# spcl/EBCC

Measured on AMD Instinct MI355X. Metric: fp32 GB/s encode+decode, 721x1440 ERA5 frames MAX_ERROR=0.5, higher is better.
Workload: dtype f32; 1 GPU; 256-frame batch 721x1440 fp32 per GPU, base_cr=30 MAX_ERROR=0.5 (BASELINE configs[1]); frames_per_gpu=256, parallelism=frames sharded over 1 GPU(s), no collective, hw_queues=4, encode_slices=3

## Files before the change

### ebcc_amd/csrc/j2k.hip

```cpp
#include <algorithm>
#include <cstring>
#include <vector>

#include "../../include/ebcc_hip.h"
#include "engine.hpp"
#include "j2k.hpp"
#include "search.hpp"

namespace ebcc {

bool j2k_create(ebcc_hip_ctx *ctx)
{
    J2kBuffers *jb = new J2kBuffers();
    ctx->j2k = jb;
    const int period = ctx->tile_period;
    std::vector<std::vector<J2kBlock>> tile_blocks((size_t) period);
    int stride = 0;
    for (int k = 0; k < period; k++) {
        jb->geoms.push_back(make_j2k_geom(ctx->height, ctx->width, tile_blocks[(size_t) k], k * ctx->height));
        stride = std::max(stride, jb->geoms.back().nblocks);
    }
    for (J2kGeom &t : jb->geoms) { t.period = period; t.stride = stride; }
    jb->geom = jb->geoms[0];
    const J2kGeom &g = jb->geom;
// ... 39 lines not shown
    ok &= (jb->cand_npass = (int *) ctx_alloc<int32_t>(ctx, 2 * F * (size_t) stride)) != nullptr;
    ok &= (jb->cand_sel = (int *) ctx_alloc<int32_t>(ctx, F)) != nullptr;
    ok &= (jb->have_rate = (int *) ctx_alloc<int32_t>(ctx, F)) != nullptr;
    ok &= (jb->rate_path = (int *) ctx_alloc<int32_t>(ctx, F * 1536 * 3)) != nullptr;
    ok &= (jb->rate_path_n = (int *) ctx_alloc<int32_t>(ctx, 2 * F)) != nullptr;
    {
        int nodes = 0;
        for (const J2kGeom &t : jb->geoms) nodes = std::max(nodes, t.tree_nodes);
        J2kBuffers::RateCache &rc = jb->rate_cache;
        rc.nodes_cap = (nodes + 3) & ~3;
        rc.cap = stride * kJ2kMaxPasses;
        rc.ok = jb->rate_path_n ? jb->rate_path_n + F : nullptr;
        ok &= (rc.mnmx = ctx_alloc<double>(ctx, F * 2)) != nullptr;
        ok &= (rc.mval = (short *) ctx_alloc<uint16_t>(ctx, F * (size_t) rc.nodes_cap)) != nullptr;
        ok &= (rc.off = (int *) ctx_alloc<int32_t>(ctx, F * (size_t) (stride + 1))) != nullptr;
        ok &= (rc.crate = ctx_alloc<uint16_t>(ctx, F * (size_t) rc.cap)) != nullptr;
        ok &= (rc.cdisto = ctx_alloc<double>(ctx, F * (size_t) rc.cap)) != nullptr;
    }
    ok &= (jb->rates = (int *) ctx_alloc<int32_t>(ctx, groups * 64 * kJ2kMaxPasses)) != nullptr;
    ok &= (jb->disto = ctx_alloc<double>(ctx, groups * 64 * kJ2kMaxPasses)) != nullptr;
    ok &= (jb->cblk_bytes = ctx_alloc<uint8_t>(ctx, groups * 64 * kJ2kCblkBytes)) != nullptr;
    ok &= (jb->stream = ctx_alloc<uint8_t>(ctx, F * jb->stream_cap)) != nullptr;
    ok &= (jb->dec_table = (int *) ctx_alloc<int32_t>(ctx, groups * 64 * 4)) != nullptr;
    ok &= (jb->dec_order = (int *) ctx_alloc<int32_t>(ctx, groups * 64 + 128)) != nullptr;
    ok &= (jb->mq_order = (int *) ctx_alloc<int32_t>(ctx, groups * 64 + 256)) != nullptr;
    ok &= (jb->jf = (J2kFrame *) ctx_alloc<uint8_t>(ctx, sizeof(J2kFrame) * F)) != nullptr;
    ok &= (jb->partial = ctx_alloc<double>(ctx, F * kPartials)) != nullptr;
    ok &= (jb->partial_u = ctx_alloc<unsigned long long>(ctx, F * kPartials)) != nullptr;
    if (!ok) return false;
    poison_alloc(jb->cblk_bytes, groups * 64 * kJ2kCblkBytes);
    poison_alloc(jb->stream, F * jb->stream_cap);
    if (stride >= 65535) { set_error("too many code-blocks"); return false; }
// ... 643 lines not shown
```

### ebcc_amd/csrc/j2k.hpp

```cpp
#pragma once

#include <vector>

#include "../../include/ebcc_hip.h"
#include "common.hpp"
#include "residual.hpp"

namespace ebcc {

constexpr int kJ2kRes = 6;
constexpr int kJ2kBands = 3 * kJ2kRes - 2;
constexpr int kJ2kMaxPlanes = 26;
constexpr int kJ2kMaxPasses = 3 * kJ2kMaxPlanes;
constexpr int kJ2kCblkBytes = 16 * 1024;
constexpr int kT1StateWords = 66 + 4 * 64;

struct J2kBand {
    int res, orient, level;
    int x0, y0, x1, y1;
    int offx, offy;
    int ncw, nch;
    int first_block;
    int expn, mant, numbps;
    float step_enc, step_dec;
// ... 95 lines not shown
    int *npass;
    float *cand_cr;
    int *cand_out;
    int *cand_npass;
    int *cand_sel;
    int *have_rate;
    int *rate_path;
    int *rate_path_n;
    struct RateCache {
        int *ok;
        double *mnmx;
        short *mval;
        int *off;
        unsigned short *crate;
        double *cdisto;
        int nodes_cap, cap;
    } rate_cache;
    uint8_t *cblk_bytes;
    uint8_t *stream;
    size_t stream_cap;
    int32_t *V;
    int *dec_table;
    int *dec_order;
    int *mq_order;
    J2kFrame *jf;
    FrameState *fs;
    double *partial;
    unsigned long long *partial_u;
};

enum T1Kernel { T1_ENCODE = 0, T1_MQ = 1, T1_RESUME = 2, T1_DECODE = 3 };
int t1_lanes_per_wave(int kernel, int total_blocks = 0);
// ... 37 lines not shown
    J2kBoxList list{};
    float *out = nullptr;
};
bool j2k_list_check(const char *who, const J2kGeom &g, size_t n_frames, const ebcc_hip_placed_box *boxes, size_t n_boxes, size_t out_floats,
                    uint8_t *keep = nullptr, J2kBoxEntry *table = nullptr, J2kPlacement *place = nullptr, int first_fused = kJ2kRes,
                    int *max_rows = nullptr, int *max_cols = nullptr);
bool j2k_boxes_as_placed(const char *who, const ebcc_hip_box *boxes, size_t n_boxes, size_t rows, size_t cols,
                         std::vector<ebcc_hip_placed_box> &placed, size_t *out_floats);
int j2k_selfcheck_div65535();

void launch_input_stats(const float *data, int n_frames, size_t n_pix, FrameState *fs, hipStream_t s);
void launch_j2k_analysis(const float *data, const J2kBuffers &jb, int n_frames, hipStream_t s);
void launch_j2k_tier1(const J2kBuffers &jb, int n_frames, hipStream_t s, bool single_kernel);
bool j2k_tier1_retry(const J2kBuffers &jb, int n_frames, const J2kFrame *host_jf, hipStream_t s);
void launch_j2k_rate(const J2kBuffers &jb, int n_frames, const int *d_active, hipStream_t s, const int *have_rate = nullptr);
void j2k_probe_hist_dump(const char *what);
void launch_j2k_rate_candidates(const J2kBuffers &jb, int n_frames, const int *d_active, hipStream_t s);
void launch_j2k_rate_publish(const J2kBuffers &jb, int n_frames, hipStream_t s);
void launch_j2k_write(const J2kBuffers &jb, int n_frames, const int *d_active, hipStream_t s);
void launch_j2k_probe_decode(const float *data, const J2kBuffers &jb, int n_frames, const int *d_active, hipStream_t s,
                             int keep_field = 1);
void launch_j2k_decode(const J2kBuffers &jb, int n_frames, hipStream_t s, const int *host_table = nullptr, const J2kRegion &region = J2kRegion{});
void launch_j2k_box_levels(const J2kBuffers &jb, int n_frames, const J2kBoxList &boxes, float *out, hipStream_t s);
void launch_j2k_fill_placed(const J2kBuffers &jb, const J2kBoxList &boxes, float *out, hipStream_t s);
void plan_decode_lanes(const int *host_table, int total, int out[4]);

}
```

### ebcc_amd/csrc/j2k_analysis.hip

```cpp
#include <array>
#include <mutex>
#include <cmath>
#include <cstdlib>
#include <vector>

#include "j2k.hpp"
#include "t1_core.hpp"
#include "t1_device.hpp"

namespace ebcc {

static int ceildivpow2(int a, int b) { return (int) (((long long) a + (1ll << b) - 1) >> b); }
static int floorlog2i(int a) { int l = 0; while (a > 1) { a >>= 1; l++; } return l; }

static const double kNormsReal[4][10] = {
    {1.000, 1.965, 4.177, 8.403, 16.90, 33.84, 67.69, 135.3, 270.6, 540.9},
    {2.022, 3.989, 8.355, 17.04, 34.27, 68.63, 137.3, 274.6, 549.0},
    {2.022, 3.989, 8.355, 17.04, 34.27, 68.63, 137.3, 274.6, 549.0},
    {2.080, 3.865, 8.307, 17.18, 34.71, 69.59, 139.3, 278.6, 557.2}};

int t1_lanes_per_wave(int kernel, int total_blocks)
{
    int t[4] = {64, 64, 4, 2};
    if (const char *e = getenv("EBCC_T1_LPW")) {
// ... 1551 lines not shown
            EBCC_HIP_CHECK(hipMemsetAsync(counters, 0, 2 * kMqClasses * sizeof(int), s));
            hipLaunchKernelGGL(k_mq_hist, dim3(ceil_div(total, 256)), dim3(256), 0, s, jb.lanerows, counters, total, (uint32_t) jb.sym_rows);
            hipLaunchKernelGGL(k_mq_offsets, dim3(1), dim3(kMqClasses), 0, s, counters);
            hipLaunchKernelGGL(k_mq_place, dim3(ceil_div((int) (groups * 64), 256)), dim3(256), 0, s, jb.lanerows, counters, jb.mq_order, total, (int) (groups * 64),
                               (uint32_t) jb.sym_rows);
            order = jb.mq_order;
        }
        hipLaunchKernelGGL(k_t1_mqrows, dim3((unsigned) groups), dim3(128), 0, s, jb.SYM, jb.lanerows, jb.blkmax, jb.cblk_len, jb.rates,
                           jb.cblk_bytes, jb.ckpt, jb.d_geom, jb.d_blocks, fs, jb.jf, total, (uint32_t) jb.sym_rows, order);
        timing_end("t1_mq", s);
    }
    timing_end("t1_encode", s);
    hipLaunchKernelGGL(k_distortion, dim3(g.stride, n_frames), dim3(256), 0, s, jb.Q6, jb.SPS, jb.numbps, jb.totalpasses,
                       jb.disto, nmsedec_luts(s), jb.d_geom, jb.d_blocks, fs);
    EBCC_HIP_LAUNCH_CHECK();
}

bool j2k_tier1_retry(const J2kBuffers &jb, int n_frames, const J2kFrame *host_jf, hipStream_t s)
{
    bool need = false;
    for (int f = 0; f < n_frames; f++) need |= (host_jf[f].overflow & 2) != 0;
    if (!need) return false;
    hipLaunchKernelGGL(k_jf_reset, dim3(ceil_div(n_frames, 64)), dim3(64), 0, s, jb.jf, n_frames);
    launch_j2k_tier1(jb, n_frames, s, true);
    return true;
}

constexpr int kFwdT = 64;
__global__ __launch_bounds__(kFwdT) void k_j2k_cols_fwd_top(const float *__restrict__ data, float *__restrict__ B, const J2kGeom *geom,
                                                             const FrameState *fs)
// ... 204 lines not shown
```

### ebcc_amd/csrc/j2k_rate.hip

```cpp
#include <cfloat>
#include <cmath>
#include <cstdlib>
#include <mutex>

#include "j2k.hpp"
#include "t1_core.hpp"
#include "t1_device.hpp"

namespace ebcc {

int j2k_inverse_dwt(float *B, const int32_t *V, const float *data, const J2kBuffers &jb, int n_frames, const FrameState *fs,
                    const int *active, hipStream_t s, int keep_field, const J2kWindow *win = nullptr, float *win_out = nullptr);

namespace {

constexpr int kMainHeaderBytes = 135;
constexpr int kRateTrieNodes = 1536;
#ifndef EBCC_RATE_THREADS
#define EBCC_RATE_THREADS 512
#endif
constexpr int kRateThreads = EBCC_RATE_THREADS;
constexpr int kWriteThreads = 256;

__device__ inline int floorlog2d(int a) { return a > 1 ? 31 - __clz(a) : 0; }
// ... 77 lines not shown
                int inc = floorlog2d(seglen) + 1 - (3 + floorlog2d(n));
                if (inc < 0) inc = 0;
                for (int k = 0; k < inc; k++) bio.bit(1);
                bio.bit(0);
                bio.bits((unsigned) seglen, 3 + inc + floorlog2d(n));
                bytes += seglen;
            }
    }
    bio.flush();
    *body = bytes;
    return bio.n;
}

__host__ __device__ inline size_t rate_off_bytes(int nblocks) { return ((size_t) (nblocks + 1) * 4 + 15) & ~(size_t) 15; }
__host__ __device__ inline size_t rate_path_bytes(int nblocks) { return (size_t) nblocks * 2 * 8 * 3 + (((size_t) nblocks + 7) & ~(size_t) 7); }

__host__ __device__ inline size_t rate_lds_bytes(int nblocks, int nodes)
{
    return 2 * ((((size_t) nblocks * 2 + 7) / 8) * 8) + (size_t) nodes * 16 + (size_t) nblocks * 20 + 128;
}

struct RateLds {
    short *npass;
    Trees t;
    short *mval0;
    short *prev;
    int *firstinc;
    unsigned int *raw;
    int *leafbits;
    __device__ static size_t bytes(int nblocks, int nodes)
// ... 80 lines not shown
}

struct PassTab {
    const int *rates;
    const double *disto;
    const __attribute__((address_space(3))) double *l_disto;
    const __attribute__((address_space(3))) unsigned short *l_rate;
    const __attribute__((address_space(3))) int *l_off;
    bool lds;
    template <bool LDS> __device__ int rate(int base, int p) const { if constexpr (LDS) return l_rate[base + p]; else return rates[base + p]; }
    template <bool LDS> __device__ double dist(int base, int p) const { if constexpr (LDS) return l_disto[base + p]; else return disto[base + p]; }
    template <bool LDS> __device__ int base_of(int b) const { if constexpr (LDS) return l_off[b]; else return b * kJ2kMaxPasses; }
};

template <bool LDS>
__device__ inline int walk_block(const PassTab &pt, const int *totalpasses, int gid0, int b, double thresh, unsigned long long &m0,
                                 unsigned long long &m1, int from = 0, int n_in = 0)
{
    if (from == 0) m0 = m1 = 0;
    int tp;
    if constexpr (LDS) tp = pt.l_off[b + 1] - pt.l_off[b]; else tp = totalpasses[gid0 + b];
    const int base = pt.base_of<LDS>(b);
    int n = n_in;
    if (thresh < 0) return tp;
    int rbase = 0;
    double dbase = 0;
    if (n_in > 0) { rbase = pt.rate<LDS>(base, n_in - 1); dbase = pt.dist<LDS>(base, n_in - 1); }
    for (int p = from; p < tp; p++) {
        const int rp = pt.rate<LDS>(base, p);
        const double dp = pt.dist<LDS>(base, p);
        unsigned int dr;
        double dd;
        if (n == 0) { dr = (unsigned int) rp; dd = dp; }
        else { dr = (unsigned int) (rp - rbase); dd = dp - dbase; }
        bool take;
        if (!dr) take = dd != 0;
        else {
            const double tdr = thresh * (double) dr;
            if (dd >= tdr * 1.00000000001) take = true;
            else if (thresh >= 1e-4 && dd <= tdr * 0.99999999999) take = false;
            else take = thresh - (dd / dr) < DBL_EPSILON;
        }
        if (take) {
            n = p + 1; rbase = rp; dbase = dp;
            if (p < 64) m0 |= 1ull << p; else m1 |= 1ull << (p - 64);
        }
    }
    return n;
}

__device__ inline double next_up(double x)
{
    long long u = __double_as_longlong(x);
    if (x == 0.0) return __longlong_as_double(1ll);
    u += x > 0.0 ? 1 : -1;
    return __longlong_as_double(u);
}
__device__ inline double next_down(double x) { return -next_up(-x); }
__device__ inline double take_limit(double s)
{
    double t = s + DBL_EPSILON;
    for (int k = 0; k < 8 && (t - s) < DBL_EPSILON; k++) t = next_up(t);
    for (int k = 0; k < 8; k++) { const double d = next_down(t); if ((d - s) < DBL_EPSILON) break; t = d; }
    return t;
}
template <bool LDS>
__device__ inline void walk_interval(const PassTab &pt, const int *totalpasses, int gid0, int b, unsigned long long m0, unsigned long long m1,
                                     int from, int n_in, double tlo, double thi, double &A, double &B)
{
    int tp;
    if constexpr (LDS) tp = pt.l_off[b + 1] - pt.l_off[b]; else tp = totalpasses[gid0 + b];
    const int base = pt.base_of<LDS>(b);
    int n = n_in, rbase = 0;
    double dbase = 0;
    if (n_in > 0) { rbase = pt.rate<LDS>(base, n_in - 1); dbase = pt.dist<LDS>(base, n_in - 1); }
    A = -DBL_MAX; B = DBL_MAX;
    const bool coarse = tlo >= 1e-4;
    for (int p = from; p < tp; p++) {
        const int rp = pt.rate<LDS>(base, p);
        const double dp = pt.dist<LDS>(base, p);
        const unsigned int dr = n == 0 ? (unsigned int) rp : (unsigned int) (rp - rbase);
        const double dd = n == 0 ? dp : dp - dbase;
        const bool taken = p < 64 ? (m0 >> p) & 1ull : (m1 >> (p - 64)) & 1ull;
        if (dr) {
            const double fdr = (double) dr;
            if (coarse && dd > thi * fdr * 1.000000001) {
                if (!taken) A = DBL_MAX;
            } else if (coarse && dd < tlo * fdr * 0.999999999) {
                if (taken) B = -DBL_MAX;
            } else {
                const double lim = take_limit(dd / fdr);
                if (taken) B = lim < B ? lim : B; else A = lim > A ? lim : A;
            }
        } else if (taken != (dd != 0)) { A = DBL_MAX; B = -DBL_MAX; }
        if (taken) { n = p + 1; rbase = rp; dbase = dp; }
    }
}

template <int NT, bool LDS>
__device__ void make_layer_impl(const J2kGeom &g, RateLds &L, const int *totalpasses, const PassTab &pt, int gid0, double thresh, int lane,
                                unsigned long long *path, const unsigned char *frozen)
{
    for (int b = lane; b < g.nblocks; b += NT) {
        if (frozen && frozen[b]) continue;
        unsigned long long m0, m1;
        const int n = walk_block<LDS>(pt, totalpasses, gid0, b, thresh, m0, m1);
        L.npass[b] = (short) n;
        if (path) { path[b] = m0; path[g.nblocks + b] = m1; }
    }
    __syncthreads();
}

template <int NT>
__device__ void make_layer(const J2kGeom &g, RateLds &L, const int *totalpasses, const PassTab &pt, int gid0, double thresh, int lane,
                           unsigned long long *path = nullptr, const unsigned char *frozen = nullptr)
{
    if (pt.lds) make_layer_impl<NT, true>(g, L, totalpasses, pt, gid0, thresh, lane, path, frozen);
    else make_layer_impl<NT, false>(g, L, totalpasses, pt, gid0, thresh, lane, path, frozen);
}

template <int NT>
// ... 141 lines not shown
            }
            if (found < 0) { count += (T - p + 7) >> 3; break; }
            count += found + 1 + 1;
            p += 8 * (found + 1) + 7;
            if (p >= T) break;
        }
        if (hdr_out && wl == 0) hdr_out[r] = count - count_before;
    }
    if (wl == 0) atomicAdd(s_sum, body + count);
    __syncthreads();
    const int total = *s_sum;
    __syncthreads();
    return total;
}

__global__ __launch_bounds__(kRateThreads) void k_rate(const int *__restrict__ numbps, const int *__restrict__ totalpasses,
                                                        const int *__restrict__ rates, const double *__restrict__ disto,
                                                        int *__restrict__ npass_out, const J2kGeom *geom, J2kFrame *jf,
                                                        const FrameState *fs, const int *active, int pass_capacity,
                                                        int *__restrict__ path_bytes, int *__restrict__ path_n,
                                                        const float *cand_cr, int *cand_out, size_t cand_stride, const int *have_rate,
                                                        J2kBuffers::RateCache cache)
{
    extern __shared__ unsigned char lds_raw[];
    __shared__ int s_sum, s_changed;
#ifdef EBCC_RATE_PROFILE
    const long long t_start = wall_clock64();
#endif
    __shared__ double s_min[kRateThreads / 64], s_max[kRateThreads / 64];
    __shared__ double s_td[5];
// ... 26 lines not shown
        for (int i = lane; i < g.tree_nodes; i += kRateThreads) L.mval0[i] = c_mval[i];
        __syncthreads();
    } else {
        trees_static<kRateThreads>(g, L, numbps, gid0, lane);
        if (record) for (int i = lane; i < g.tree_nodes; i += kRateThreads) c_mval[i] = L.mval0[i];
    }
#ifdef EBCC_RATE_PROFILE
    t_s[1] = wall_clock64() - t_start;
#endif
    for (int b = lane; b < g.nblocks; b += kRateThreads) L.prev[b] = -1;
    __shared__ int s_fit;
    unsigned char *extra = lds_raw + ((rate_lds_bytes(g.nblocks, g.tree_nodes) + 15) & ~(size_t) 15);
    int *l_off = (int *) extra;
    unsigned long long *p_cur = (unsigned long long *) (extra + rate_off_bytes(g.nblocks));
    unsigned long long *p_lo = p_cur + 2 * g.nblocks, *p_hi = p_lo + 2 * g.nblocks;
    unsigned char *frozen = (unsigned char *) (p_hi + 2 * g.nblocks);
    double *l_disto = (double *) (frozen + (((size_t) g.nblocks + 7) & ~(size_t) 7));
    for (int b = lane; b < g.nblocks; b += kRateThreads) frozen[b] = 0;
    if (cached) {
        for (int b = lane; b <= g.nblocks; b += kRateThreads) l_off[b] = c_off[b];
        if (lane == 0) { const int running = c_off[g.nblocks]; s_fit = running <= pass_capacity ? running : -1; }
    } else {
        __shared__ int s_scan[kRateThreads / 64];
        int running = 0;
        for (int base = 0; base < g.nblocks; base += kRateThreads) {
            const int b = base + lane;
            const int tp = b < g.nblocks ? totalpasses[gid0 + b] : 0;
            int x = tp;
            for (int d = 1; d < 64; d <<= 1) { const int y = __shfl_up(x, d); if ((lane & 63) >= d) x += y; }
            if ((lane & 63) == 63) s_scan[lane >> 6] = x;
            __syncthreads();
            int before = running, tot = 0;
            for (int w = 0; w < kRateThreads / 64; w++) { const int v = s_scan[w]; if (w < (lane >> 6)) before += v; tot += v; }
            if (b < g.nblocks) l_off[b] = before + x - tp;
            running += tot;
            __syncthreads();
        }
        if (lane == 0) { l_off[g.nblocks] = running; s_fit = running <= pass_capacity ? running : -1; }
        __syncthreads();
        if (record) for (int b = lane; b <= g.nblocks; b += kRateThreads) c_off[b] = l_off[b];
    }
    __syncthreads();
#ifdef EBCC_RATE_PROFILE
    t_s[2] = wall_clock64() - t_start;
#endif
    const int n_entries = s_fit;
    unsigned short *l_rate = (unsigned short *) (l_disto + (n_entries > 0 ? n_entries : 0));
    typedef __attribute__((address_space(3))) double lds_double;
    typedef __attribute__((address_space(3))) int lds_int;
    typedef __attribute__((address_space(3))) unsigned short lds_ushort;
    PassTab pt{rates + (size_t) gid0 * kJ2kMaxPasses, disto + (size_t) gid0 * kJ2kMaxPasses, (const lds_double *) l_disto,
               (const lds_ushort *) l_rate, (const lds_int *) l_off, n_entries >= 0};
    if (pt.lds && cached) {
// ... 6 lines not shown
            const int r_ = pt.rates[idx];
            const double d_ = pt.disto[idx];
            const int b = idx / kJ2kMaxPasses, p = idx - b * kJ2kMaxPasses;
            const int o = l_off[b];
            if (p < l_off[b + 1] - o) {
                l_rate[o + p] = (unsigned short) r_;
                l_disto[o + p] = d_;
                if (record) { c_rate[o + p] = (unsigned short) r_; c_disto[o + p] = d_; }
            }
        }
        __syncthreads();
    }
#ifdef EBCC_RATE_PROFILE
    t_s[3] = wall_clock64() - t_start;
#endif
    int prev_bytes = 0;
    auto sized = [&]() -> int {
        if (lane == 0) s_changed = 0;
        __syncthreads();
        int ch = 0;
        for (int b = lane; b < g.nblocks; b += kRateThreads) { if (L.prev[b] != L.npass[b]) ch = 1; L.prev[b] = L.npass[b]; }
        if (ch) s_changed = 1;
        __syncthreads();
        if (s_changed) {
#ifdef EBCC_RATE_CHECK
            const int ref = layer_bytes<kRateThreads>(g, L, rates, gid0, lane, &s_sum);
            prev_bytes = layer_bytes_fast<kRateThreads>(g, L, rates, gid0, lane, &s_sum);
            if (ref != prev_bytes && lane == 0) { printf("rate check: frame %d fast %d serial %d\n", frame, prev_bytes, ref); }
            prev_bytes = ref;
#else
// ... 28 lines not shown
            if (sl > mx) mx = sl;
        }
    }
    for (int d = 32; d >= 1; d >>= 1) {
        const double omn = __shfl_xor(mn, d), omx = __shfl_xor(mx, d);
        mn = omn < mn ? omn : mn; mx = omx > mx ? omx : mx;
    }
    if ((lane & 63) == 0) { s_min[lane >> 6] = mn; s_max[lane >> 6] = mx; }
    __syncthreads();
    for (int i = 0; i < kRateThreads / 64; i++) { mn = s_min[i] < mn ? s_min[i] : mn; mx = s_max[i] > mx ? s_max[i] : mx; }
    if (record) {
        __threadfence();
        __syncthreads();
        if (lane == 0) {
            cache.mnmx[2 * frame] = mn; cache.mnmx[2 * frame + 1] = mx;
            if (pt.lds) { __threadfence(); __hip_atomic_store(&cache.ok[frame], 1, __ATOMIC_RELEASE, __HIP_MEMORY_SCOPE_AGENT); }
        }
    }
    }

#ifdef EBCC_RATE_PROFILE
    long long t_setup = wall_clock64() - t_start, t_ml = 0, t_sz = 0, t_replay_end = 0, t_tail = 0, t_loop_end = 0; int n_it = 0, n_real = 0, n_replayed = 0, n_tail = 0;
#define RP_T0 const long long rp0 = wall_clock64()
#define RP_ADD(acc) acc += wall_clock64() - rp0
#else
#define RP_T0
#define RP_ADD(acc)
#endif
    double good = -1;
    bool converged = false;
    if (rate > 0.0f) {
// ... 14 lines not shown
#ifdef EBCC_RATE_PROFILE
                n_replayed++;
#endif
                const int bytes = trie[3 * cur];
                const int f = (long long) bytes <= maxlen;
                if (f) { hi = thresh; stable = thresh; bytes_hi = bytes; hi_from_rec = true; hi_seen = false; }
                else { lo = thresh; bytes_lo = bytes; lo_from_rec = true; lo_seen = false; }
                parent = cur; pdir = f;
                const int nxt = trie[3 * cur + 1 + f];
                cur = nxt > 0 ? nxt : -1;
                continue;
            }
#ifdef EBCC_RATE_PROFILE
            if (!t_replay_end) t_replay_end = wall_clock64();
#endif
            if (hi_from_rec) { make_layer<kRateThreads>(g, L, totalpasses, pt, gid0, hi, lane, p_hi); hi_seen = true; hi_from_rec = false; }
            if (lo_from_rec) { make_layer<kRateThreads>(g, L, totalpasses, pt, gid0, lo, lane, p_lo); lo_seen = true; lo_from_rec = false; }
            { RP_T0; make_layer<kRateThreads>(g, L, totalpasses, pt, gid0, thresh, lane, p_cur, frozen); RP_ADD(t_ml); }
            if (lane == 0) s_nun = 0;
            int at_lo = lo_seen, at_hi = hi_seen;
            for (int b = lane; b < g.nblocks; b += kRateThreads) {
                if (frozen[b]) continue;
                if (p_cur[b] != p_lo[b] || p_cur[g.nblocks + b] != p_lo[g.nblocks + b]) at_lo = 0;
                if (p_cur[b] != p_hi[b] || p_cur[g.nblocks + b] != p_hi[g.nblocks + b]) at_hi = 0;
            }
            at_lo = __syncthreads_and(at_lo);
            at_hi = __syncthreads_and(at_hi);
            int bytes;
            if (at_lo) bytes = bytes_lo;
            else if (at_hi) bytes = bytes_hi;
            else { RP_T0; bytes = sized(); RP_ADD(t_sz); }
#ifdef EBCC_RATE_PROFILE
            n_it++; n_real += (at_lo || at_hi) ? 0 : s_changed;
#endif
            const bool fits = (long long) bytes <= maxlen;
            if (record && n_nodes < kRateTrieNodes && (parent >= 0 || n_nodes == 0)) {
                if (lane == 0) {
                    trie[3 * n_nodes] = bytes; trie[3 * n_nodes + 1] = 0; trie[3 * n_nodes + 2] = 0;
                    if (parent >= 0) trie[3 * parent + 1 + pdir] = n_nodes;
                    path_n[frame] = n_nodes + 1;
                }
                parent = n_nodes++; pdir = fits;
            } else {
                parent = -1;
            }
            if (fits) bytes_hi = bytes; else bytes_lo = bytes;
            if (fits) { hi = thresh; stable = thresh; hi_seen = true; } else { lo = thresh; lo_seen = true; }
            unsigned long long *end = fits ? p_hi : p_lo;
            int same = lo_seen && hi_seen;
            for (int b = lane; b < g.nblocks; b += kRateThreads) {
                if (frozen[b]) continue;
                end[b] = p_cur[b]; end[g.nblocks + b] = p_cur[g.nblocks + b];
                if (lo_seen && hi_seen && p_lo[b] == p_hi[b] && p_lo[g.nblocks + b] == p_hi[g.nblocks + b]) frozen[b] = 1;
                else {
                    same = 0;
                    const int k = atomicAdd(&s_nun, 1);
                    if (k < 64) s_list[k] = b;
                }
            }
            if (__syncthreads_and(same)) { converged = true; break; }
            if (lo_seen && hi_seen && s_nun <= 64) {
                RP_T0;
                if (lane < 64) {
                    const int nb = g.nblocks, b = lane < s_nun ? s_list[lane] : -1;
                    double tlo = lo, thi = hi, tprev = prev, tstable = stable, tthresh = thresh;
                    int ti = i, tn = n_nodes, tparent = parent, tpdir = pdir, status = 0;
                    int from = 0, n_in = 0;
                    unsigned long long c0 = 0, c1 = 0;
                    if (b >= 0) {
                        const unsigned long long d0 = p_lo[b] ^ p_hi[b], d1 = p_lo[nb + b] ^ p_hi[nb + b];
                        from = d0 ? __builtin_ctzll(d0) : (d1 ? 64 + __builtin_ctzll(d1) : 0);
                        if (from > 0) {
                            c0 = from >= 64 ? p_lo[b] : p_lo[b] & ((1ull << from) - 1ull);
                            c1 = from > 64 ? p_lo[nb + b] & ((1ull << (from - 64)) - 1ull) : 0ull;
                            n_in = c1 ? 128 - __builtin_clzll(c1) : (c0 ? 64 - __builtin_clzll(c0) : 0);
                        }
                    }
                    double a_lo = -DBL_MAX, b_lo = DBL_MAX, a_hi = -DBL_MAX, b_hi = DBL_MAX;
                    if (b >= 0) {
                        if (pt.lds) {
                            walk_interval<true>(pt, totalpasses, gid0, b, p_lo[b], p_lo[nb + b], from, n_in, tlo, thi, a_lo, b_lo);
                            walk_interval<true>(pt, totalpasses, gid0, b, p_hi[b], p_hi[nb + b], from, n_in, tlo, thi, a_hi, b_hi);
                        } else {
                            walk_interval<false>(pt, totalpasses, gid0, b, p_lo[b], p_lo[nb + b], from, n_in, tlo, thi, a_lo, b_lo);
                            walk_interval<false>(pt, totalpasses, gid0, b, p_hi[b], p_hi[nb + b], from, n_in, tlo, thi, a_hi, b_hi);
                        }
                    }
                    (void) c0; (void) c1;
                    for (int j = i + 1; j < 128; j++) {
                        const double t = (tlo + thi) / 2;
                        if (t == tprev) { tthresh = t; break; }
                        const int all_lo = __all(b < 0 || (t >= a_lo && t < b_lo));
                        const int all_hi = __all(b < 0 || (t >= a_hi && t < b_hi));
                        if (!all_lo && !all_hi) { status = 1; break; }
                        tthresh = t; tprev = t; ti = j;
                        const int bytes = all_lo ? bytes_lo : bytes_hi;
                        const bool fits = (long long) bytes <= maxlen;
                        if (record && tn < kRateTrieNodes && (tparent >= 0 || tn == 0)) {
                            if (lane == 0) {
                                trie[3 * tn] = bytes; trie[3 * tn + 1] = 0; trie[3 * tn + 2] = 0;
// ... 16 lines not shown
                i = s_ti[0]; n_nodes = s_ti[1]; parent = s_ti[2]; pdir = s_ti[3];
                const int status = s_ti[4];
                __syncthreads();
                RP_ADD(t_tail);
#ifdef EBCC_RATE_PROFILE
                n_tail++;
#endif
                if (status == 0) break;
            }
        }
        good = stable == 0 ? thresh : stable;
    }
#ifdef EBCC_RATE_PROFILE
    t_loop_end = wall_clock64();
#endif
    if (!converged) make_layer<kRateThreads>(g, L, totalpasses, pt, gid0, good, lane);
    const int body = sized();
    for (int b = lane; b < g.nblocks; b += kRateThreads) npass_out[gid0 + b] = L.npass[b];
    if (lane == 0 && candidate) {
        int *o = cand_out + (size_t) (2 * frame + slot) * 3;
        o[0] = body; o[1] = kMainHeaderBytes + 12 + 2 + body + 2; o[2] = (int) (rate > 0.0f ? ceil((double) rate) : 0);
    }
    if (lane == 0 && !candidate) {
        jf[frame].body_bytes = body;
        jf[frame].stream_bytes = kMainHeaderBytes + 12 + 2 + body + 2;
        jf[frame].maxlen = (int) (rate > 0.0f ? ceil((double) rate) : 0);
#ifdef EBCC_RATE_PROFILE
        if (frame == 0) printf("k_rate frame0 setup: entry %lld, trees %lld, offsets %lld, tables %lld us\n", t_s[0] / 100, t_s[1] / 100, t_s[2] / 100, t_s[3] / 100);
        if (frame == 0) printf("k_rate frame0: setup %lld us, %d replayed steps until %lld us, make_layer %lld us, sized %lld us, computed iterations %d (real sizings %d), tail %lld us in %d visits, loop ends at %lld us, total %lld us\n",
                               t_setup / 100, n_replayed, t_replay_end ? (t_replay_end - t_start) / 100 : -1, t_ml / 100, t_sz / 100, n_it, n_real, t_tail / 100, n_tail,
                               (t_loop_end - t_start) / 100, (wall_clock64() - t_start) / 100);
// ... 534 lines not shown
    t1::decode_resume(st, DecSrc{cblk_bytes + (size_t) gid * kJ2kCblkBytes, len}, blk.w, blk.h, geom->bands[blk.band].orient, P,
                      np, r, stripe, ck, tab, ctxp);
}

size_t rate_lds(const J2kBuffers &jb)
{
    size_t n = 0;
    for (const J2kGeom &g : jb.geoms) n = std::max(n, rate_lds_bytes(g.nblocks, g.tree_nodes));
    return n;
}

}

static void rate_launch(const J2kBuffers &jb, int n_frames, const int *d_active, hipStream_t s, bool candidates, const int *have_rate)
{
    const size_t head = ((rate_lds(jb) + 15) & ~(size_t) 15) + rate_off_bytes(jb.geom.stride) + rate_path_bytes(jb.geom.stride);
    const size_t budget = 150 * 1024;
    size_t want = (size_t) jb.geom.stride * kJ2kMaxPasses;
    if (head + want * 10 + 16 > budget) want = head + 16 < budget ? (budget - head - 16) / 10 : 0;
    const size_t lds = head + want * 10 + 16;
    static std::once_flag once;
    std::call_once(once, [] {
        EBCC_HIP_CHECK(hipFuncSetAttribute((const void *) k_rate, hipFuncAttributeMaxDynamicSharedMemorySize, 150 * 1024));
    });
    hipLaunchKernelGGL(k_rate, dim3(n_frames, candidates ? 2 : 1), dim3(kRateThreads), lds, s, jb.numbps, jb.totalpasses, jb.rates,
                       jb.disto, candidates ? jb.cand_npass : jb.npass, jb.d_geom, jb.jf, jb.fs, d_active, (int) want, jb.rate_path, jb.rate_path_n,
                       candidates ? jb.cand_cr : nullptr, jb.cand_out, (size_t) jb.max_frames * (size_t) jb.geom.stride, have_rate, jb.rate_cache);
    EBCC_HIP_LAUNCH_CHECK();
}

void launch_j2k_rate(const J2kBuffers &jb, int n_frames, const int *d_active, hipStream_t s, const int *have_rate)
{
    ScopedTiming t("rate_alloc", s);
    rate_launch(jb, n_frames, d_active, s, false, have_rate);
}

void launch_j2k_rate_candidates(const J2kBuffers &jb, int n_frames, const int *d_active, hipStream_t s)
{
    rate_launch(jb, n_frames, d_active, s, true, nullptr);
}

__global__ void k_rate_publish(const int *sel, const int *cand_npass, const int *cand_out, size_t cand_stride, int *npass, J2kFrame *jf,
// ... 196 lines not shown
```

Measured before the change: 8.830 GB/s.

## Precompute per-block threshold tables for rate allocation and binary-search them

Adds a k_rate_tables kernel, launched after distortion, that walks each code-block's rate/distortion passes once. It records the threshold breakpoints at which the number of included passes changes, along with the pass count at each. The rate-allocation bisection then looks up each block's pass count by binary search in this table. This replaces re-walking every pass at every threshold iteration, and bracket indices narrow the search. The old walk path stays behind an environment variable; the cost is an extra kernel launch, extra global memory for the tables, and subtle exactness risks in the breakpoint computation.

```diff
diff --git a/ebcc_amd/csrc/j2k.hip b/ebcc_amd/csrc/j2k.hip
--- a/ebcc_amd/csrc/j2k.hip
+++ b/ebcc_amd/csrc/j2k.hip
@@ -77,8 +77,20 @@
         ok &= (rc.mnmx = ctx_alloc<double>(ctx, F * 2)) != nullptr;
         ok &= (rc.mval = (short *) ctx_alloc<uint16_t>(ctx, F * (size_t) rc.nodes_cap)) != nullptr;
         ok &= (rc.off = (int *) ctx_alloc<int32_t>(ctx, F * (size_t) (stride + 1))) != nullptr;
-        ok &= (rc.crate = ctx_alloc<uint16_t>(ctx, F * (size_t) rc.cap)) != nullptr;
-        ok &= (rc.cdisto = ctx_alloc<double>(ctx, F * (size_t) rc.cap)) != nullptr;
+        const char *e = getenv("EBCC_HIP_RATE_WALK");
+        jb->rate_walk = e && atoi(e);
+        rc.crate = nullptr; rc.cdisto = nullptr; rc.wlim = nullptr; rc.wnp = nullptr; rc.wcnt = nullptr;
+        if (jb->rate_walk) {
+            ok &= (rc.crate = ctx_alloc<uint16_t>(ctx, F * (size_t) rc.cap)) != nullptr;
+            ok &= (rc.cdisto = ctx_alloc<double>(ctx, F * (size_t) rc.cap)) != nullptr;
+        } else {
+            const size_t cnt_bytes = (F * (size_t) stride * sizeof(uint16_t) + 15) & ~(size_t) 15;
+            uint8_t *small = nullptr;
+            ok &= (rc.wlim = ctx_alloc<double>(ctx, F * (size_t) (rc.cap + stride))) != nullptr;
+            ok &= (small = ctx_alloc<uint8_t>(ctx, cnt_bytes + F * (size_t) (rc.cap + stride))) != nullptr;
+            rc.wcnt = (unsigned short *) small;
+            rc.wnp = small ? small + cnt_bytes : nullptr;
+        }
     }
     ok &= (jb->rates = (int *) ctx_alloc<int32_t>(ctx, groups * 64 * kJ2kMaxPasses)) != nullptr;
     ok &= (jb->disto = ctx_alloc<double>(ctx, groups * 64 * kJ2kMaxPasses)) != nullptr;
diff --git a/ebcc_amd/csrc/j2k.hpp b/ebcc_amd/csrc/j2k.hpp
--- a/ebcc_amd/csrc/j2k.hpp
+++ b/ebcc_amd/csrc/j2k.hpp
@@ -133,8 +133,12 @@
         int *off;
         unsigned short *crate;
         double *cdisto;
+        double *wlim;
+        unsigned char *wnp;
+        unsigned short *wcnt;
         int nodes_cap, cap;
     } rate_cache;
+    bool rate_walk;
     uint8_t *cblk_bytes;
     uint8_t *stream;
     size_t stream_cap;
@@ -202,6 +206,7 @@
 void launch_j2k_tier1(const J2kBuffers &jb, int n_frames, hipStream_t s, bool single_kernel);
 bool j2k_tier1_retry(const J2kBuffers &jb, int n_frames, const J2kFrame *host_jf, hipStream_t s);
 void launch_j2k_rate(const J2kBuffers &jb, int n_frames, const int *d_active, hipStream_t s, const int *have_rate = nullptr);
+void launch_j2k_rate_tables(const J2kBuffers &jb, int n_frames, hipStream_t s);
 void j2k_probe_hist_dump(const char *what);
 void launch_j2k_rate_candidates(const J2kBuffers &jb, int n_frames, const int *d_active, hipStream_t s);
 void launch_j2k_rate_publish(const J2kBuffers &jb, int n_frames, hipStream_t s);
diff --git a/ebcc_amd/csrc/j2k_analysis.hip b/ebcc_amd/csrc/j2k_analysis.hip
--- a/ebcc_amd/csrc/j2k_analysis.hip
+++ b/ebcc_amd/csrc/j2k_analysis.hip
@@ -1589,6 +1589,7 @@
     hipLaunchKernelGGL(k_distortion, dim3(g.stride, n_frames), dim3(256), 0, s, jb.Q6, jb.SPS, jb.numbps, jb.totalpasses,
                        jb.disto, nmsedec_luts(s), jb.d_geom, jb.d_blocks, fs);
     EBCC_HIP_LAUNCH_CHECK();
+    launch_j2k_rate_tables(jb, n_frames, s);
 }
 
 bool j2k_tier1_retry(const J2kBuffers &jb, int n_frames, const J2kFrame *host_jf, hipStream_t s)
diff --git a/ebcc_amd/csrc/j2k_rate.hip b/ebcc_amd/csrc/j2k_rate.hip
--- a/ebcc_amd/csrc/j2k_rate.hip
+++ b/ebcc_amd/csrc/j2k_rate.hip
@@ -4,6 +4,7 @@
 #include <mutex>
 
 #include "j2k.hpp"
+#include "rate_walk.hpp"
 #include "t1_core.hpp"
 #include "t1_device.hpp"
 
@@ -115,6 +116,7 @@
 
 __host__ __device__ inline size_t rate_off_bytes(int nblocks) { return ((size_t) (nblocks + 1) * 4 + 15) & ~(size_t) 15; }
 __host__ __device__ inline size_t rate_path_bytes(int nblocks) { return (size_t) nblocks * 2 * 8 * 3 + (((size_t) nblocks + 7) & ~(size_t) 7); }
+__host__ __device__ inline size_t rate_index_bytes(int nblocks) { return (((size_t) nblocks * 2 * 3 + 7) & ~(size_t) 7) + (((size_t) nblocks + 7) & ~(size_t) 7); }
 
 __host__ __device__ inline size_t rate_lds_bytes(int nblocks, int nodes)
 {
@@ -225,88 +227,15 @@
 };
 
 template <bool LDS>
-__device__ inline int walk_block(const PassTab &pt, const int *totalpasses, int gid0, int b, double thresh, unsigned long long &m0,
-                                 unsigned long long &m1, int from = 0, int n_in = 0)
-{
-    if (from == 0) m0 = m1 = 0;
-    int tp;
-    if constexpr (LDS) tp = pt.l_off[b + 1] - pt.l_off[b]; else tp = totalpasses[gid0 + b];
-    const int base = pt.base_of<LDS>(b);
-    int n = n_in;
-    if (thresh < 0) return tp;
-    int rbase = 0;
-    double dbase = 0;
-    if (n_in > 0) { rbase = pt.rate<LDS>(base, n_in - 1); dbase = pt.dist<LDS>(base, n_in - 1); }
-    for (int p = from; p < tp; p++) {
-        const int rp = pt.rate<LDS>(base, p);
-        const double dp = pt.dist<LDS>(base, p);
-        unsigned int dr;
-        double dd;
-        if (n == 0) { dr = (unsigned int) rp; dd = dp; }
-        else { dr = (unsigned int) (rp - rbase); dd = dp - dbase; }
-        bool take;
-        if (!dr) take = dd != 0;
-        else {
-            const double tdr = thresh * (double) dr;
-            if (dd >= tdr * 1.00000000001) take = true;
-            else if (thresh >= 1e-4 && dd <= tdr * 0.99999999999) take = false;
-            else take = thresh - (dd / dr) < DBL_EPSILON;
-        }
-        if (take) {
-            n = p + 1; rbase = rp; dbase = dp;
-            if (p < 64) m0 |= 1ull << p; else m1 |= 1ull << (p - 64);
-        }
-    }
-    return n;
-}
-
-__device__ inline double next_up(double x)
-{
-    long long u = __double_as_longlong(x);
-    if (x == 0.0) return __longlong_as_double(1ll);
-    u += x > 0.0 ? 1 : -1;
-    return __longlong_as_double(u);
-}
-__device__ inline double next_down(double x) { return -next_up(-x); }
-__device__ inline double take_limit(double s)
-{
-    double t = s + DBL_EPSILON;
-    for (int k = 0; k < 8 && (t - s) < DBL_EPSILON; k++) t = next_up(t);
-    for (int k = 0; k < 8; k++) { const double d = next_down(t); if ((d - s) < DBL_EPSILON) break; t = d; }
-    return t;
-}
-template <bool LDS>
-__device__ inline void walk_interval(const PassTab &pt, const int *totalpasses, int gid0, int b, unsigned long long m0, unsigned long long m1,
-                                     int from, int n_in, double tlo, double thi, double &A, double &B)
-{
-    int tp;
-    if constexpr (LDS) tp = pt.l_off[b + 1] - pt.l_off[b]; else tp = totalpasses[gid0 + b];
-    const int base = pt.base_of<LDS>(b);
-    int n = n_in, rbase = 0;
-    double dbase = 0;
-    if (n_in > 0) { rbase = pt.rate<LDS>(base, n_in - 1); dbase = pt.dist<LDS>(base, n_in - 1); }
-    A = -DBL_MAX; B = DBL_MAX;
-    const bool coarse = tlo >= 1e-4;
-    for (int p = from; p < tp; p++) {
-        const int rp = pt.rate<LDS>(base, p);
-        const double dp = pt.dist<LDS>(base, p);
-        const unsigned int dr = n == 0 ? (unsigned int) rp : (unsigned int) (rp - rbase);
-        const double dd = n == 0 ? dp : dp - dbase;
-        const bool taken = p < 64 ? (m0 >> p) & 1ull : (m1 >> (p - 64)) & 1ull;
-        if (dr) {
-            const double fdr = (double) dr;
-            if (coarse && dd > thi * fdr * 1.000000001) {
-                if (!taken) A = DBL_MAX;
-            } else if (coarse && dd < tlo * fdr * 0.999999999) {
-                if (taken) B = -DBL_MAX;
-            } else {
-                const double lim = take_limit(dd / fdr);
-                if (taken) B = lim < B ? lim : B; else A = lim > A ? lim : A;
-            }
-        } else if (taken != (dd != 0)) { A = DBL_MAX; B = -DBL_MAX; }
-        if (taken) { n = p + 1; rbase = rp; dbase = dp; }
-    }
-}
+struct PassView {
+    const PassTab &pt;
+    const int *totalpasses;
+    int gid0;
+    __device__ int passes(int b) const { if constexpr (LDS) return pt.l_off[b + 1] - pt.l_off[b]; else return totalpasses[gid0 + b]; }
+    __device__ int base_of(int b) const { return pt.template base_of<LDS>(b); }
+    __device__ int rate(int base, int p) const { return pt.template rate<LDS>(base, p); }
+    __device__ double dist(int base, int p) const { return pt.template dist<LDS>(base, p); }
+};
 
 template <int NT, bool LDS>
 __device__ void make_layer_impl(const J2kGeom &g, RateLds &L, const int *totalpasses, const PassTab &pt, int gid0, double thresh, int lane,
@@ -315,7 +244,7 @@
     for (int b = lane; b < g.nblocks; b += NT) {
         if (frozen && frozen[b]) continue;
         unsigned long long m0, m1;
-        const int n = walk_block<LDS>(pt, totalpasses, gid0, b, thresh, m0, m1);
+        const int n = walk_block(PassView<LDS>{pt, totalpasses, gid0}, b, thresh, m0, m1);
         L.npass[b] = (short) n;
         if (path) { path[b] = m0; path[g.nblocks + b] = m1; }
     }
@@ -487,6 +416,57 @@
     return total;
 }
 
+constexpr int kTableLanes = 64;
+constexpr size_t kTableLds = (size_t) kTableLanes * kJ2kMaxPasses * 10;
+
+struct PassColumn {
+    const __attribute__((address_space(3))) double *d;
+    const __attribute__((address_space(3))) unsigned short *r;
+    int tp;
+    __device__ int passes(int) const { return tp; }
+    __device__ int base_of(int) const { return 0; }
+    __device__ int rate(int, int p) const { return r[p * kTableLanes]; }
+    __device__ double dist(int, int p) const { return d[p * kTableLanes]; }
+};
+
+__global__ __launch_bounds__(kTableLanes) void k_rate_tables(const int *__restrict__ totalpasses, const int *__restrict__ rates,
+                                                              const double *__restrict__ disto, const J2kGeom *geom,
+                                                              const FrameState *fs, J2kBuffers::RateCache cache)
+{
+    extern __shared__ unsigned char lds_raw[];
+    const int frame = blockIdx.y, lane = threadIdx.x;
+    if (fs[frame].const_field) return;
+    const J2kGeom &g = j2k_frame_geom(geom, frame);
+    const int gid0 = frame * g.stride, b0 = blockIdx.x * kTableLanes;
+    if (b0 >= g.nblocks) return;
+    auto passes_of = [&](int b) { return b < g.nblocks ? min(max(totalpasses[gid0 + b], 0), kJ2kMaxPasses) : 0; };
+    int before = 0;
+    for (int c = 0; c < b0; c += kTableLanes) before += passes_of(c + lane);
+    for (int d = 32; d >= 1; d >>= 1) before += __shfl_xor(before, d);
+    const int b = b0 + lane, tp = passes_of(b);
+    int x = tp;
+    for (int d = 1; d < 64; d <<= 1) { const int y = __shfl_up(x, d); if (lane >= d) x += y; }
+    before += x - tp;
+    double *l_disto = (double *) lds_raw;
+    unsigned short *l_rate = (unsigned short *) (l_disto + kTableLanes * kJ2kMaxPasses);
+    for (int i = 0; i < kTableLanes && b0 + i < g.nblocks; i++) {
+        const int n = __shfl(tp, i);
+        const size_t row = (size_t) (gid0 + b0 + i) * kJ2kMaxPasses;
+        for (int p = lane; p < n; p += kTableLanes) {
+            l_rate[p * kTableLanes + i] = (unsigned short) rates[row + p];
+            l_disto[p * kTableLanes + i] = disto[row + p];
+        }
+    }
+    __syncthreads();
+    if (b >= g.nblocks) return;
+    typedef __attribute__((address_space(3))) double lds_double;
+    typedef __attribute__((address_space(3))) unsigned short lds_ushort;
+    const PassColumn col{(const lds_double *) l_disto + lane, (const lds_ushort *) l_rate + lane, tp};
+    const size_t o = (size_t) frame * (size_t) (cache.cap + g.stride) + (size_t) (before + b);
+    cache.wcnt[gid0 + b] = (unsigned short) walk_table_build(col, 0, cache.wlim + o, cache.wnp + o, tp + 1);
+}
+
+template <bool TAB>
 __global__ __launch_bounds__(kRateThreads) void k_rate(const int *__restrict__ numbps, const int *__restrict__ totalpasses,
                                                         const int *__restrict__ rates, const double *__restrict__ disto,
                                                         int *__restrict__ npass_out, const J2kGeom *geom, J2kFrame *jf,
@@ -543,12 +523,17 @@
     int *l_off = (int *) extra;
     unsigned long long *p_cur = (unsigned long long *) (extra + rate_off_bytes(g.nblocks));
     unsigned long long *p_lo = p_cur + 2 * g.nblocks, *p_hi = p_lo + 2 * g.nblocks;
-    unsigned char *frozen = (unsigned char *) (p_hi + 2 * g.nblocks);
+    constexpr unsigned short kNoWalk = 0xFFFFu;
+    unsigned short *i_cur = (unsigned short *) p_cur, *i_lo = i_cur + g.nblocks, *i_hi = i_lo + g.nblocks;
+    unsigned char *frozen = TAB ? (unsigned char *) p_cur + (((size_t) g.nblocks * 2 * 3 + 7) & ~(size_t) 7) : (unsigned char *) (p_hi + 2 * g.nblocks);
     double *l_disto = (double *) (frozen + (((size_t) g.nblocks + 7) & ~(size_t) 7));
+    const double *const w_lim = TAB ? cache.wlim + (size_t) frame * (size_t) (cache.cap + g.stride) : nullptr;
+    const unsigned char *const w_np = TAB ? cache.wnp + (size_t) frame * (size_t) (cache.cap + g.stride) : nullptr;
+    const unsigned short *const w_cnt = TAB ? cache.wcnt + gid0 : nullptr;
     for (int b = lane; b < g.nblocks; b += kRateThreads) frozen[b] = 0;
     if (cached) {
         for (int b = lane; b <= g.nblocks; b += kRateThreads) l_off[b] = c_off[b];
-        if (lane == 0) { const int running = c_off[g.nblocks]; s_fit = running <= pass_capacity ? running : -1; }
+        if (lane == 0) { const int running = c_off[g.nblocks]; s_fit = !TAB && running <= pass_capacity ? running : -1; }
     } else {
         __shared__ int s_scan[kRateThreads / 64];
         int running = 0;
@@ -565,7 +550,7 @@
             running += tot;
             __syncthreads();
         }
-        if (lane == 0) { l_off[g.nblocks] = running; s_fit = running <= pass_capacity ? running : -1; }
+        if (lane == 0) { l_off[g.nblocks] = running; s_fit = !TAB && running <= pass_capacity ? running : -1; }
         __syncthreads();
         if (record) for (int b = lane; b <= g.nblocks; b += kRateThreads) c_off[b] = l_off[b];
     }
@@ -602,6 +587,24 @@
 #ifdef EBCC_RATE_PROFILE
     t_s[3] = wall_clock64() - t_start;
 #endif
+    auto lookup_layer = [&](double thresh, unsigned short *idx, bool set_npass, bool skip_frozen, bool bracket, bool lo_known, bool hi_known) {
+        for (int b = lane; b < g.nblocks; b += kRateThreads) {
+            if (skip_frozen && frozen[b]) continue;
+            const int o = l_off[b] + b, cnt = w_cnt[b];
+            int a = 0, z = cnt - 1;
+            if (bracket && hi_known && i_hi[b] != kNoWalk) a = i_hi[b];
+            if (bracket && lo_known && i_lo[b] != kNoWalk) z = i_lo[b];
+            const int k = thresh < 0 ? -1 : walk_table_find(w_lim + o, a, z, thresh);
+            if (idx) idx[b] = k < 0 ? kNoWalk : (unsigned short) k;
+            if (set_npass) {
+                int n;
+                if (k >= 0) n = w_np[o + k];
+                else { unsigned long long m0, m1; n = walk_block(PassView<false>{pt, totalpasses, gid0}, b, thresh, m0, m1); }
+                L.npass[b] = (short) n;
+            }
+        }
+        __syncthreads();
+    };
     int prev_bytes = 0;
     auto sized = [&]() -> int {
         if (lane == 0) s_changed = 0;
@@ -660,7 +663,7 @@
         __syncthreads();
         if (lane == 0) {
             cache.mnmx[2 * frame] = mn; cache.mnmx[2 * frame + 1] = mx;
-            if (pt.lds) { __threadfence(); __hip_atomic_store(&cache.ok[frame], 1, __ATOMIC_RELEASE, __HIP_MEMORY_SCOPE_AGENT); }
+            if (TAB || pt.lds) { __threadfence(); __hip_atomic_store(&cache.ok[frame], 1, __ATOMIC_RELEASE, __HIP_MEMORY_SCOPE_AGENT); }
         }
     }
     }
@@ -705,13 +708,24 @@
 #ifdef EBCC_RATE_PROFILE
             if (!t_replay_end) t_replay_end = wall_clock64();
 #endif
+            if constexpr (TAB) {
+                if (hi_from_rec) { lookup_layer(hi, i_hi, false, false, false, false, false); hi_seen = true; hi_from_rec = false; }
+                if (lo_from_rec) { lookup_layer(lo, i_lo, false, false, false, false, false); lo_seen = true; lo_from_rec = false; }
+                { RP_T0; lookup_layer(thresh, i_cur, true, true, true, lo_seen, hi_seen); RP_ADD(t_ml); }
+            } else {
             if (hi_from_rec) { make_layer<kRateThreads>(g, L, totalpasses, pt, gid0, hi, lane, p_hi); hi_seen = true; hi_from_rec = false; }
             if (lo_from_rec) { make_layer<kRateThreads>(g, L, totalpasses, pt, gid0, lo, lane, p_lo); lo_seen = true; lo_from_rec = false; }
             { RP_T0; make_layer<kRateThreads>(g, L, totalpasses, pt, gid0, thresh, lane, p_cur, frozen); RP_ADD(t_ml); }
+            }
             if (lane == 0) s_nun = 0;
             int at_lo = lo_seen, at_hi = hi_seen;
             for (int b = lane; b < g.nblocks; b += kRateThreads) {
                 if (frozen[b]) continue;
+                if constexpr (TAB) {
+                    if (i_cur[b] == kNoWalk || i_cur[b] != i_lo[b]) at_lo = 0;
+                    if (i_cur[b] == kNoWalk || i_cur[b] != i_hi[b]) at_hi = 0;
+                    continue;
+                }
                 if (p_cur[b] != p_lo[b] || p_cur[g.nblocks + b] != p_lo[g.nblocks + b]) at_lo = 0;
                 if (p_cur[b] != p_hi[b] || p_cur[g.nblocks + b] != p_hi[g.nblocks + b]) at_hi = 0;
             }
@@ -738,11 +752,19 @@
             if (fits) bytes_hi = bytes; else bytes_lo = bytes;
             if (fits) { hi = thresh; stable = thresh; hi_seen = true; } else { lo = thresh; lo_seen = true; }
             unsigned long long *end = fits ? p_hi : p_lo;
+            unsigned short *i_end = fits ? i_hi : i_lo;
             int same = lo_seen && hi_seen;
             for (int b = lane; b < g.nblocks; b += kRateThreads) {
                 if (frozen[b]) continue;
-                end[b] = p_cur[b]; end[g.nblocks + b] = p_cur[g.nblocks + b];
-                if (lo_seen && hi_seen && p_lo[b] == p_hi[b] && p_lo[g.nblocks + b] == p_hi[g.nblocks + b]) frozen[b] = 1;
+                bool settled;
+                if constexpr (TAB) {
+                    i_end[b] = i_cur[b];
+                    settled = lo_seen && hi_seen && i_lo[b] == i_hi[b] && i_lo[b] != kNoWalk;
+                } else {
+                    end[b] = p_cur[b]; end[g.nblocks + b] = p_cur[g.nblocks + b];
+                    settled = lo_seen && hi_seen && p_lo[b] == p_hi[b] && p_lo[g.nblocks + b] == p_hi[g.nblocks + b];
+                }
+                if (settled) frozen[b] = 1;
                 else {
                     same = 0;
                     const int k = atomicAdd(&s_nun, 1);
@@ -758,7 +780,7 @@
                     int ti = i, tn = n_nodes, tparent = parent, tpdir = pdir, status = 0;
                     int from = 0, n_in = 0;
                     unsigned long long c0 = 0, c1 = 0;
-                    if (b >= 0) {
+                    if (!TAB && b >= 0) {
                         const unsigned long long d0 = p_lo[b] ^ p_hi[b], d1 = p_lo[nb + b] ^ p_hi[nb + b];
                         from = d0 ? __builtin_ctzll(d0) : (d1 ? 64 + __builtin_ctzll(d1) : 0);
                         if (from > 0) {
@@ -768,13 +790,20 @@
                         }
                     }
                     double a_lo = -DBL_MAX, b_lo = DBL_MAX, a_hi = -DBL_MAX, b_hi = DBL_MAX;
-                    if (b >= 0) {
+                    if (TAB && b >= 0) {
+                        const double *wl = w_lim + l_off[b] + b;
+                        const int klo = i_lo[b], khi = i_hi[b];
+                        if (klo != kNoWalk) { a_lo = wl[klo]; b_lo = klo > 0 ? wl[klo - 1] : DBL_MAX; } else { a_lo = DBL_MAX; b_lo = -DBL_MAX; }
+                        if (khi != kNoWalk) { a_hi = wl[khi]; b_hi = khi > 0 ? wl[khi - 1] : DBL_MAX; } else { a_hi = DBL_MAX; b_hi = -DBL_MAX; }
+                    } else if (b >= 0) {
                         if (pt.lds) {
-                            walk_interval<true>(pt, totalpasses, gid0, b, p_lo[b], p_lo[nb + b], from, n_in, tlo, thi, a_lo, b_lo);
-                            walk_interval<true>(pt, totalpasses, gid0, b, p_hi[b], p_hi[nb + b], from, n_in, tlo, thi, a_hi, b_hi);
+                            const PassView<true> pv{pt, totalpasses, gid0};
+                            walk_interval(pv, b, p_lo[b], p_lo[nb + b], from, n_in, tlo, thi, a_lo, b_lo);
+                            walk_interval(pv, b, p_hi[b], p_hi[nb + b], from, n_in, tlo, thi, a_hi, b_hi);
                         } else {
-                            walk_interval<false>(pt, totalpasses, gid0, b, p_lo[b], p_lo[nb + b], from, n_in, tlo, thi, a_lo, b_lo);
-                            walk_interval<false>(pt, totalpasses, gid0, b, p_hi[b], p_hi[nb + b], from, n_in, tlo, thi, a_hi, b_hi);
+                            const PassView<false> pv{pt, totalpasses, gid0};
+                            walk_interval(pv, b, p_lo[b], p_lo[nb + b], from, n_in, tlo, thi, a_lo, b_lo);
+                            walk_interval(pv, b, p_hi[b], p_hi[nb + b], from, n_in, tlo, thi, a_hi, b_hi);
                         }
                     }
                     (void) c0; (void) c1;
@@ -821,7 +850,10 @@
 #ifdef EBCC_RATE_PROFILE
     t_loop_end = wall_clock64();
 #endif
-    if (!converged) make_layer<kRateThreads>(g, L, totalpasses, pt, gid0, good, lane);
+    if (!converged) {
+        if constexpr (TAB) lookup_layer(good, nullptr, true, false, false, false, false);
+        else make_layer<kRateThreads>(g, L, totalpasses, pt, gid0, good, lane);
+    }
     const int body = sized();
     for (int b = lane; b < g.nblocks; b += kRateThreads) npass_out[gid0 + b] = L.npass[b];
     if (lane == 0 && candidate) {
@@ -1386,18 +1418,33 @@
 
 static void rate_launch(const J2kBuffers &jb, int n_frames, const int *d_active, hipStream_t s, bool candidates, const int *have_rate)
 {
-    const size_t head = ((rate_lds(jb) + 15) & ~(size_t) 15) + rate_off_bytes(jb.geom.stride) + rate_path_bytes(jb.geom.stride);
+    const size_t carve = ((rate_lds(jb) + 15) & ~(size_t) 15) + rate_off_bytes(jb.geom.stride);
     const size_t budget = 150 * 1024;
-    size_t want = (size_t) jb.geom.stride * kJ2kMaxPasses;
-    if (head + want * 10 + 16 > budget) want = head + 16 < budget ? (budget - head - 16) / 10 : 0;
-    const size_t lds = head + want * 10 + 16;
     static std::once_flag once;
     std::call_once(once, [] {
-        EBCC_HIP_CHECK(hipFuncSetAttribute((const void *) k_rate, hipFuncAttributeMaxDynamicSharedMemorySize, 150 * 1024));
+        EBCC_HIP_CHECK(hipFuncSetAttribute((const void *) k_rate<false>, hipFuncAttributeMaxDynamicSharedMemorySize, 150 * 1024));
+        EBCC_HIP_CHECK(hipFuncSetAttribute((const void *) k_rate<true>, hipFuncAttributeMaxDynamicSharedMemorySize, 150 * 1024));
     });
-    hipLaunchKernelGGL(k_rate, dim3(n_frames, candidates ? 2 : 1), dim3(kRateThreads), lds, s, jb.numbps, jb.totalpasses, jb.rates,
-                       jb.disto, candidates ? jb.cand_npass : jb.npass, jb.d_geom, jb.jf, jb.fs, d_active, (int) want, jb.rate_path, jb.rate_path_n,
-                       candidates ? jb.cand_cr : nullptr, jb.cand_out, (size_t) jb.max_frames * (size_t) jb.geom.stride, have_rate, jb.rate_cache);
+    size_t want = 0, lds = carve + rate_index_bytes(jb.geom.stride) + 16;
+    if (jb.rate_walk) {
+        const size_t head = carve + rate_path_bytes(jb.geom.stride);
+        want = (size_t) jb.geom.stride * kJ2kMaxPasses;
+        if (head + want * 10 + 16 > budget) want = head + 16 < budget ? (budget - head - 16) / 10 : 0;
+        lds = head + want * 10 + 16;
+    }
+    hipLaunchKernelGGL(jb.rate_walk ? k_rate<false> : k_rate<true>, dim3(n_frames, candidates ? 2 : 1), dim3(kRateThreads), lds, s, jb.numbps,
+                       jb.totalpasses, jb.rates, jb.disto, candidates ? jb.cand_npass : jb.npass, jb.d_geom, jb.jf, jb.fs, d_active, (int) want,
+                       jb.rate_path, jb.rate_path_n, candidates ? jb.cand_cr : nullptr, jb.cand_out,
+                       (size_t) jb.max_frames * (size_t) jb.geom.stride, have_rate, jb.rate_cache);
+    EBCC_HIP_LAUNCH_CHECK();
+}
+
+void launch_j2k_rate_tables(const J2kBuffers &jb, int n_frames, hipStream_t s)
+{
+    if (jb.rate_walk) return;
+    ScopedTiming t("rate_alloc", s);
+    hipLaunchKernelGGL(k_rate_tables, dim3(ceil_div(jb.geom.stride, kTableLanes), n_frames), dim3(kTableLanes), kTableLds, s, jb.totalpasses,
+                       jb.rates, jb.disto, jb.d_geom, jb.fs, jb.rate_cache);
     EBCC_HIP_LAUNCH_CHECK();
 }
 
diff --git a/ebcc_amd/csrc/rate_walk.hpp b/ebcc_amd/csrc/rate_walk.hpp
--- /dev/null
+++ b/ebcc_amd/csrc/rate_walk.hpp
@@ -0,0 +1,177 @@
+#pragma once
+#include <cfloat>
+
+#if defined(__HIPCC__)
+#define EBCC_RW_HD __host__ __device__
+#else
+#define EBCC_RW_HD
+#endif
+
+namespace ebcc {
+
+template <class Tab>
+EBCC_RW_HD inline int walk_block(const Tab &pt, int b, double thresh, unsigned long long &m0, unsigned long long &m1, int from = 0,
+                                 int n_in = 0)
+{
+    if (from == 0) m0 = m1 = 0;
+    const int tp = pt.passes(b);
+    const int base = pt.base_of(b);
+    int n = n_in;
+    if (thresh < 0) return tp;
+    int rbase = 0;
+    double dbase = 0;
+    if (n_in > 0) { rbase = pt.rate(base, n_in - 1); dbase = pt.dist(base, n_in - 1); }
+    for (int p = from; p < tp; p++) {
+        const int rp = pt.rate(base, p);
+        const double dp = pt.dist(base, p);
+        unsigned int dr;
+        double dd;
+        if (n == 0) { dr = (unsigned int) rp; dd = dp; }
+        else { dr = (unsigned int) (rp - rbase); dd = dp - dbase; }
+        bool take;
+        if (!dr) take = dd != 0;
+        else {
+            const double tdr = thresh * (double) dr;
+            if (dd >= tdr * 1.00000000001) take = true;
+            else if (thresh >= 1e-4 && dd <= tdr * 0.99999999999) take = false;
+            else take = thresh - (dd / dr) < DBL_EPSILON;
+        }
+        if (take) {
+            n = p + 1; rbase = rp; dbase = dp;
+            if (p < 64) m0 |= 1ull << p; else m1 |= 1ull << (p - 64);
+        }
+    }
+    return n;
+}
+
+EBCC_RW_HD inline double next_up(double x)
+{
+    if (x == 0.0) { const long long one = 1; double r; __builtin_memcpy(&r, &one, 8); return r; }
+    long long u;
+    __builtin_memcpy(&u, &x, 8);
+    u += x > 0.0 ? 1 : -1;
+    double r;
+    __builtin_memcpy(&r, &u, 8);
+    return r;
+}
+EBCC_RW_HD inline double next_down(double x) { return -next_up(-x); }
+EBCC_RW_HD inline double take_limit(double s)
+{
+    double t = s + DBL_EPSILON;
+    for (int k = 0; k < 8 && (t - s) < DBL_EPSILON; k++) t = next_up(t);
+    for (int k = 0; k < 8; k++) { const double d = next_down(t); if ((d - s) < DBL_EPSILON) break; t = d; }
+    return t;
+}
+template <class Tab>
+EBCC_RW_HD inline void walk_interval(const Tab &pt, int b, unsigned long long m0, unsigned long long m1, int from, int n_in, double tlo,
+                                     double thi, double &A, double &B)
+{
+    const int tp = pt.passes(b);
+    const int base = pt.base_of(b);
+    int n = n_in, rbase = 0;
+    double dbase = 0;
+    if (n_in > 0) { rbase = pt.rate(base, n_in - 1); dbase = pt.dist(base, n_in - 1); }
+    A = -DBL_MAX; B = DBL_MAX;
+    const bool coarse = tlo >= 1e-4;
+    for (int p = from; p < tp; p++) {
+        const int rp = pt.rate(base, p);
+        const double dp = pt.dist(base, p);
+        const unsigned int dr = n == 0 ? (unsigned int) rp : (unsigned int) (rp - rbase);
+        const double dd = n == 0 ? dp : dp - dbase;
+        const bool taken = p < 64 ? (m0 >> p) & 1ull : (m1 >> (p - 64)) & 1ull;
+        if (dr) {
+            const double fdr = (double) dr;
+            if (coarse && dd > thi * fdr * 1.000000001) {
+                if (!taken) A = DBL_MAX;
+            } else if (coarse && dd < tlo * fdr * 0.999999999) {
+                if (taken) B = -DBL_MAX;
+            } else {
+                const double lim = take_limit(dd / fdr);
+                if (taken) B = lim < B ? lim : B; else A = lim > A ? lim : A;
+            }
+        } else if (taken != (dd != 0)) { A = DBL_MAX; B = -DBL_MAX; }
+        if (taken) { n = p + 1; rbase = rp; dbase = dp; }
+    }
+}
+
+
+template <class Tab>
+EBCC_RW_HD inline int walk_and_limit(const Tab &pt, int b, double thresh, unsigned long long &m0, unsigned long long &m1, int known,
+                                     double &A, int &first)
+{
+    const int tp = pt.passes(b);
+    const int base = pt.base_of(b);
+    int n = 0, rbase = 0;
+    double dbase = 0;
+    double bd = 0, br = 0;
+    first = -1;
+    if (known == 0) m0 = m1 = 0;
+    for (int p = 0; p < tp; p++) {
+        const int rp = pt.rate(base, p);
+        const double dp = pt.dist(base, p);
+        unsigned int dr;
+        double dd;
+        if (n == 0) { dr = (unsigned int) rp; dd = dp; }
+        else { dr = (unsigned int) (rp - rbase); dd = dp - dbase; }
+        bool take;
+        if (p < known) take = p < 64 ? (m0 >> p) & 1ull : (m1 >> (p - 64)) & 1ull;
+        else if (!dr) take = dd != 0;
+        else {
+            const double tdr = thresh * (double) dr;
+            if (dd >= tdr * 1.00000000001) take = true;
+            else if (thresh >= 1e-4 && dd <= tdr * 0.99999999999) take = false;
+            else take = thresh - (dd / dr) < DBL_EPSILON;
+        }
+        if (take) {
+            n = p + 1; rbase = rp; dbase = dp;
+            if (p < 64) m0 |= 1ull << p; else m1 |= 1ull << (p - 64);
+            continue;
+        }
+        if (!dr) continue;
+        const double fdr = (double) dr;
+        if (br == 0) { bd = dd; br = fdr; first = p; continue; }
+        if (bd >= 1e-4 * br) {
+            const double l = dd * br, r = bd * fdr;
+            if (l < r * 0.999999999) continue;
+            if (l > r * 1.000000001) { bd = dd; br = fdr; first = p; continue; }
+        }
+        if (take_limit(dd / fdr) > take_limit(bd / br)) { bd = dd; br = fdr; first = p; }
+    }
+    A = br != 0 ? take_limit(bd / br) : -DBL_MAX;
+    return n;
+}
+
+template <class Tab>
+EBCC_RW_HD inline int walk_table_build(const Tab &pt, int b, double *lim, unsigned char *np, int max_n)
+{
+    double t = DBL_MAX;
+    int count = 0, known = 0;
+    unsigned long long m0 = 0, m1 = 0;
+    while (count < max_n) {
+        double A;
+        int first;
+        const int n = walk_and_limit(pt, b, t, m0, m1, known, A, first);
+        if (!(A <= t)) break;
+        lim[count] = A; np[count] = (unsigned char) n;
+        count++;
+        if (A <= 0) break;
+        t = next_down(A);
+        m0 = first >= 64 ? m0 : m0 & ((1ull << first) - 1ull);
+        m1 = first > 64 ? m1 & ((1ull << (first - 64)) - 1ull) : 0ull;
+        if (first < 64) m0 |= 1ull << first; else m1 |= 1ull << (first - 64);
+        known = first + 1;
+    }
+    return count;
+}
+
+EBCC_RW_HD inline int walk_table_find(const double *lim, int a, int z, double t)
+{
+    if (z < a) return -1;
+    while (a < z) {
+        const int m = (a + z) >> 1;
+        if (lim[m] <= t) z = m; else a = m + 1;
+    }
+    return lim[a] <= t ? a : -1;
+}
+
+}
```

Measured after the change: 9.189 GB/s, median of 6. 1.04x the previous value.
